# tangxyw/RecAlgorithm

Hardware: NVIDIA H100
Metric: ctr_fwd_bwd_samples_per_sec (higher is better)
Workload: dtype f32

## Files before the change

### recalgorithm_b200/csrc/ctr_common.cuh

```cuda
#pragma once
#include <cuda_runtime.h>
#include <stdint.h>
#include <stdio.h>

#include <type_traits>

#include "../../include/ctr_b200.h"

namespace ctr {

void set_error(const char* fmt, ...);
void count_launch(int n = 1);
int sm_count();

#define CTR_REQUIRE(cond, ...)                                   \
  do {                                                           \
    if (!(cond)) {                                               \
      ctr::set_error(__VA_ARGS__);                               \
      return CTR_ERR_INVALID_ARG;                                \
    }                                                            \
  } while (0)

#define CTR_UNSUPPORTED(cond, ...)                               \
  do {                                                           \
    if (cond) {                                                  \
      ctr::set_error(__VA_ARGS__);                               \
      return CTR_ERR_UNSUPPORTED;                                \
    }                                                            \
  } while (0)

#define CTR_CHECK_LAUNCH(name)                                                   \
  do {                                                                           \
    cudaError_t e__ = cudaGetLastError();                                        \
    if (e__ != cudaSuccess) {                                                    \
      ctr::set_error("%s: launch failed: %s", name, cudaGetErrorString(e__));    \
      return CTR_ERR_CUDA;                                                       \
    }                                                                            \
    ctr::count_launch();                                                         \
  } while (0)

#define CTR_CUDA(call)                                                           \
  do {                                                                           \
    cudaError_t e__ = (call);                                                    \
    if (e__ != cudaSuccess) {                                                    \
      ctr::set_error("%s failed: %s", #call, cudaGetErrorString(e__));           \
      return CTR_ERR_CUDA;                                                       \
    }                                                                            \
  } while (0)

__device__ __forceinline__ float warp_sum(float v) {
#pragma unroll
  for (int o = 16; o > 0; o >>= 1) v += __shfl_xor_sync(0xffffffffu, v, o);
  return v;
}

__device__ __forceinline__ float4 ldg_stream_f4(const float4* p) {
  float4 r;
  asm volatile("ld.global.nc.L1::no_allocate.v4.f32 {%0,%1,%2,%3}, [%4];"
               : "=f"(r.x), "=f"(r.y), "=f"(r.z), "=f"(r.w) : "l"(p));
  return r;
}
__device__ __forceinline__ void stg_stream_f4(float4* p, const float4& v) {
  asm volatile("st.global.cs.v4.f32 [%0], {%1,%2,%3,%4};" ::"l"(p), "f"(v.x), "f"(v.y), "f"(v.z), "f"(v.w)
               : "memory");
}
__device__ __forceinline__ long long ldg_stream_i64(const long long* p) {
  long long r;
  asm volatile("ld.global.nc.L1::no_allocate.s64 %0, [%1];" : "=l"(r) : "l"(p));
  return r;
}

static inline cudaStream_t as_stream(void* s) { return reinterpret_cast<cudaStream_t>(s); }
static inline bool aligned16(const void* p) { return (reinterpret_cast<uintptr_t>(p) & 15u) == 0; }

static inline int capped_grid(long long need, long long cap) { return (int)(need < cap ? need : cap); }

template <class... P, class... A>
int launch(const char* what, void (*k)(P...), dim3 grid, dim3 block, size_t smem, cudaStream_t st, const A&... args) {
  if (smem > 48 * 1024) CTR_CUDA(cudaFuncSetAttribute(k, cudaFuncAttributeMaxDynamicSharedMemorySize, (int)smem));
  k<<<grid, block, smem, st>>>(args...);
  CTR_CHECK_LAUNCH(what);
  return CTR_OK;
}

template <int MAX_PER_SM = 0, class... P, class... A>
int launch_resident(const char* what, void (*k)(P...), long long need, int block, size_t smem, cudaStream_t st,
                    const A&... args) {
  if (smem > 48 * 1024) CTR_CUDA(cudaFuncSetAttribute(k, cudaFuncAttributeMaxDynamicSharedMemorySize, (int)smem));
  int per_sm = 0;
  if (cudaOccupancyMaxActiveBlocksPerMultiprocessor(&per_sm, k, block, smem) != cudaSuccess || per_sm < 1) per_sm = 1;
  if (MAX_PER_SM > 0 && per_sm > MAX_PER_SM) per_sm = MAX_PER_SM;
  k<<<capped_grid(need, (long long)per_sm * sm_count()), block, smem, st>>>(args...);
  CTR_CHECK_LAUNCH(what);
  return CTR_OK;
}

template <int... Vs, class F>
int with_const(int v, F&& f) {
  int rc = CTR_OK;
  const bool hit = ((v == Vs && ((rc = f(std::integral_constant<int, Vs>{})), true)) || ...);
  if (!hit) {
    set_error("no kernel instantiation for %d", v);
    return CTR_ERR_INVALID_ARG;
  }
  return rc;
}
template <class F>
int with_lpr(int64_t D, F&& f) {
  return with_const<1, 2, 4, 8, 16, 32>((int)(D / 4), f);
}

}
```

### recalgorithm_b200/csrc/embed_fm2.cu

```cuda
#include "lookup_bwd.cuh"

namespace ctr {

struct PeerTables {
  const float4* base[8];
  int G, logG;
};

__device__ __forceinline__ long long load_id(const long long* p) { return ldg_stream_i64(p); }
__device__ __forceinline__ long long load_id(const int* p) {
  int r;
  asm volatile("ld.global.nc.L1::no_allocate.s32 %0, [%1];" : "=r"(r) : "l"(p));
  return (long long)r;
}
__device__ __forceinline__ float4 ld_peer_f4(const float4* p) {
  float4 r;
  asm volatile("ld.global.v4.f32 {%0,%1,%2,%3}, [%4];" : "=f"(r.x), "=f"(r.y), "=f"(r.z), "=f"(r.w) : "l"(p));
  return r;
}

template <int LPR, bool SH, int MINB, bool BI = false, typename IdT = long long, bool LIN = false, bool SEQ = false>
__global__ void __launch_bounds__(256, MINB)
embed_fm2_fwd_kernel(const float4* __restrict__ table, const PeerTables peers, const long long* __restrict__ row_off,
                     const IdT* __restrict__ ids, int B, int F, float4* __restrict__ tile,
                     float* __restrict__ fm2, long long* __restrict__ ids64_out,
                     const float4* __restrict__ wlin, float* __restrict__ lin) {
  constexpr int RPW = 32 / LPR;
  constexpr int UB = LPR < 8 ? LPR : 8;
  const unsigned full = 0xffffffffu;
  const int lane = threadIdx.x & 31;
  const int sub = lane / LPR;
  const int c = lane % LPR;
  const int warp0 = (blockIdx.x * blockDim.x + threadIdx.x) >> 5;
  const int nwarps = (gridDim.x * blockDim.x) >> 5;

  for (int b = warp0; b < B; b += nwarps) {
    float4 S = f4_zero(), Q = f4_zero();
    float lin_acc = 0.f;
    for (int f0 = 0; f0 < F; f0 += 32) {
      const int nf = min(32, F - f0);
      long long row = -1;
      if (lane < nf) {
        const long long id = load_id(ids + (size_t)b * F + f0 + lane);
        const long long lo = __ldg(row_off + (SEQ ? 0 : f0 + lane)), hi = __ldg(row_off + (SEQ ? 1 : f0 + lane + 1));
        row = (id >= 0 && id < hi - lo) ? lo + id : -1;
        if (sizeof(IdT) == 4 && ids64_out != nullptr) ids64_out[(size_t)b * F + f0 + lane] = id;
      }
#pragma unroll
      for (int it0 = 0; it0 < LPR; it0 += UB) {
        if (it0 * RPW >= nf) break;
        float4 v[UB];
        bool in[UB];
#pragma unroll
        for (int u = 0; u < UB; ++u) {
          const int fs = (it0 + u) * RPW + sub;
          const long long r = __shfl_sync(full, row, fs);
          in[u] = fs < nf;
          v[u] = f4_zero();
          if (in[u] && r >= 0) {
            if (SH) v[u] = ld_peer_f4(peers.base[r & (peers.G - 1)] + (size_t)(r >> peers.logG) * LPR + c);
            else v[u] = ldg_stream_f4(table + (size_t)r * LPR + c);
          }
        }
#pragma unroll
        for (int u = 0; u < UB; ++u) {
          S.x += v[u].x; S.y += v[u].y; S.z += v[u].z; S.w += v[u].w;
          Q.x = __fadd_rn(Q.x, __fmul_rn(v[u].x, v[u].x)); Q.y = __fadd_rn(Q.y, __fmul_rn(v[u].y, v[u].y));
          Q.z = __fadd_rn(Q.z, __fmul_rn(v[u].z, v[u].z)); Q.w = __fadd_rn(Q.w, __fmul_rn(v[u].w, v[u].w));
          if (tile != nullptr && in[u]) {
            const int fs = (it0 + u) * RPW + sub;
            stg_stream_f4(tile + ((size_t)b * F + f0 + fs) * LPR + c, v[u]);
          }
          if (LIN && in[u]) {
            const float4 w = __ldg(wlin + (size_t)(f0 + (it0 + u) * RPW + sub) * LPR + c);
            lin_acc += v[u].x * w.x + v[u].y * w.y + v[u].z * w.z + v[u].w * w.w;
          }
        }
      }
    }
    if (LIN) {
      lin_acc = warp_sum(lin_acc);
      if (lane == 0) lin[b] = lin_acc;
    }
    if (fm2 != nullptr) {
#pragma unroll
      for (int o = LPR; o < 32; o <<= 1) {
        S.x += __shfl_xor_sync(full, S.x, o); S.y += __shfl_xor_sync(full, S.y, o);
        S.z += __shfl_xor_sync(full, S.z, o); S.w += __shfl_xor_sync(full, S.w, o);
        Q.x += __shfl_xor_sync(full, Q.x, o); Q.y += __shfl_xor_sync(full, Q.y, o);
        Q.z += __shfl_xor_sync(full, Q.z, o); Q.w += __shfl_xor_sync(full, Q.w, o);
      }
      if (BI) {
        if (lane < LPR) {
          float4 r;
          r.x = 0.5f * __fsub_rn(__fmul_rn(S.x, S.x), Q.x); r.y = 0.5f * __fsub_rn(__fmul_rn(S.y, S.y), Q.y);
          r.z = 0.5f * __fsub_rn(__fmul_rn(S.z, S.z), Q.z); r.w = 0.5f * __fsub_rn(__fmul_rn(S.w, S.w), Q.w);
          reinterpret_cast<float4*>(fm2)[(size_t)b * LPR + c] = r;
        }
        continue;
      }
      float p = 0.5f * __fsub_rn(__fmul_rn(S.x, S.x), Q.x) + 0.5f * __fsub_rn(__fmul_rn(S.y, S.y), Q.y) +
                0.5f * __fsub_rn(__fmul_rn(S.z, S.z), Q.z) + 0.5f * __fsub_rn(__fmul_rn(S.w, S.w), Q.w);
#pragma unroll
      for (int o = 1; o < LPR; o <<= 1) p += __shfl_xor_sync(full, p, o);
      if (lane == 0) fm2[b] = p;
    }
  }
}

enum { FM2_PLAIN, FM2_BI, FM2_LIN };

struct StoreRow {
  float4* __restrict__ o_row;
  __device__ __forceinline__ void fetch(int, int) {}
  __device__ __forceinline__ void operator()(int, int j, const float4& r) { stg_stream_f4(o_row + j, r); }
};

template <int LPR, int HOLD, int MODE>
__global__ void __launch_bounds__(256, MODE == FM2_LIN ? 2 : 0)
embed_fm2_bwd_kernel(const float4* __restrict__ tile, const float4* __restrict__ d_tile, const float* __restrict__ d_fm2,
                     const float* __restrict__ d_lin, int B, int F, float4* __restrict__ row_grads, float4* __restrict__ d_wlin) {
  extern __shared__ float4 s_lin[];
  const int lane = threadIdx.x & 31;
  const int warp0 = (blockIdx.x * blockDim.x + threadIdx.x) >> 5;
  const int nwarps = (gridDim.x * blockDim.x) >> 5;
  const int n4 = F * LPR;
  LinHead<MODE == FM2_LIN ? HOLD : 1> lin;
  if (MODE == FM2_LIN) lin.stage(s_lin, d_tile, n4);
  for (int b = warp0; b < B; b += nwarps) {
    StoreRow sink{row_grads + (size_t)b * n4};
    RowGrad rows{d_tile ? d_tile + (size_t)b * n4 : nullptr};
    float4 g4;
    if (MODE == FM2_BI) {
      g4 = __ldg(reinterpret_cast<const float4*>(d_fm2) + (size_t)b * LPR + lane % LPR);
    } else {
      const float g = d_fm2 ? __ldg(d_fm2 + b) : 0.f;
      g4 = make_float4(g, g, g, g);
    }
    if constexpr (MODE == FM2_LIN) {
      lin.gl = d_lin ? __ldg(d_lin + b) : 0.f;
      lookup_bwd_sample<LPR, HOLD>(tile + (size_t)b * n4, n4, lane, g4, lin, sink);
    } else {
      lookup_bwd_sample<LPR, HOLD>(tile + (size_t)b * n4, n4, lane, g4, rows, sink);
    }
  }
  if (MODE == FM2_LIN) lin.flush(d_wlin, lane);
}

template <int LPR>
__global__ void __launch_bounds__(256)
embed_scatter_add_kernel(float4* __restrict__ grad_table, const long long* __restrict__ row_off,
                         const long long* __restrict__ ids, const float4* __restrict__ row_grads, int B, int F) {
  const size_t total = (size_t)B * F * LPR;
  for (size_t t = (size_t)blockIdx.x * blockDim.x + threadIdx.x; t < total; t += (size_t)gridDim.x * blockDim.x) {
    const int c = (int)(t % LPR);
    const size_t bf = t / LPR;
    const int f = (int)(bf % F);
    const long long id = __ldg(ids + bf);
    const long long lo = __ldg(row_off + f), hi = __ldg(row_off + f + 1);
    if (id >= 0 && id < hi - lo) {
      const float4 g = ldg_stream_f4(row_grads + t);
      atomicAdd(grad_table + (size_t)(lo + id) * LPR + c, g);
    }
  }
}

__global__ void __launch_bounds__(256)
bag_lookup_fwd_kernel(const float* __restrict__ table, long long V, int D, const long long* __restrict__ ids,
                      const long long* __restrict__ offsets, int B, float* __restrict__ out, long long out_stride,
                      int G) {
  const int tid = blockIdx.x * blockDim.x + threadIdx.x;
  const int gl = threadIdx.x % G;
  const int nthreads = gridDim.x * blockDim.x;
  for (int b = tid / G; b < B; b += nthreads / G) {
    const long long s = __ldg(offsets + b), e = __ldg(offsets + b + 1);
    float acc[8];
#pragma unroll
    for (int k = 0; k < 8; ++k) acc[k] = 0.f;
    int n = 0;
    for (long long i = s; i < e; ++i) {
      const long long id = __ldg(ids + i);
      if (id >= 0 && id < V) {
        ++n;
#pragma unroll
        for (int k = 0; k < 8; ++k) {
          const int dd = k * G + gl;
          if (dd < D) acc[k] += __ldg(table + (size_t)id * D + dd);
        }
      }
    }
#pragma unroll
    for (int k = 0; k < 8; ++k) {
      const int dd = k * G + gl;
      if (dd < D) out[(size_t)b * out_stride + dd] = n > 0 ? acc[k] / (float)n : 0.f;
    }
  }
}

__global__ void __launch_bounds__(256)
bag_lookup_bwd_kernel(const float* __restrict__ d_out, long long out_stride, long long V, int D,
                      const long long* __restrict__ ids, const long long* __restrict__ offsets, int B,
                      float* __restrict__ row_grads, int G) {
  const int tid = blockIdx.x * blockDim.x + threadIdx.x;
  const int gl = threadIdx.x % G;
  const int nthreads = gridDim.x * blockDim.x;
  for (int b = tid / G; b < B; b += nthreads / G) {
    const long long s = __ldg(offsets + b), e = __ldg(offsets + b + 1);
    int n = 0;
    for (long long i = s; i < e; ++i) {
      const long long id = __ldg(ids + i);
      n += (id >= 0 && id < V);
    }
    for (long long i = s; i < e; ++i) {
      const long long id = __ldg(ids + i);
      const bool ok = id >= 0 && id < V;
      for (int dd = gl; dd < D; dd += G) {
        const float g = __ldg(d_out + (size_t)b * out_stride + dd);
        row_grads[(size_t)i * D + dd] = ok ? g / (float)n : 0.f;
      }
    }
  }
}

__global__ void __launch_bounds__(256)
first_order_fwd_kernel(const float* __restrict__ w, const long long* __restrict__ row_off,
                       const long long* __restrict__ ids, int B, int F, float bias, float* __restrict__ out) {
  const int lane = threadIdx.x & 31;
  const int warp0 = (blockIdx.x * blockDim.x + threadIdx.x) >> 5;
  const int nwarps = (gridDim.x * blockDim.x) >> 5;
  for (int b = warp0; b < B; b += nwarps) {
    float acc = 0.f;
    for (int f = lane; f < F; f += 32) {
      const long long id = ldg_stream_i64(ids + (size_t)b * F + f);
      const long long lo = __ldg(row_off + f), hi = __ldg(row_off + f + 1);
      if (id >= 0 && id < hi - lo) acc += __ldg(w + lo + id);
    }
    acc = warp_sum(acc);
    if (lane == 0) out[b] = acc + bias;
  }
}

template <int LPR, typename IdT>
static int launch_fwd(const float* table, const PeerTables* peers, const int64_t* off, const IdT* ids, int64_t B,
                      int64_t F, float* tile, float* fm2, int64_t* ids64_out, cudaStream_t st) {
  PeerTables none = {};
  const PeerTables& pt = peers ? *peers : none;
  auto go = [&](auto k) {
    return launch_resident("ctr_embed_fm2_fwd", k, (B + 7) / 8, 256, 0, st, reinterpret_cast<const float4*>(table), pt,
                           reinterpret_cast<const long long*>(off), ids, (int)B, (int)F, reinterpret_cast<float4*>(tile), fm2,
                           reinterpret_cast<long long*>(ids64_out), nullptr, nullptr);
  };
  return peers != nullptr ? go(embed_fm2_fwd_kernel<LPR, true, 1, false, IdT>) : go(embed_fm2_fwd_kernel<LPR, false, 4, false, IdT>);
}

template <int MODE>
static int launch_bwd(const char* what, const float* tile, const float* d_tile, const float* d_fm2, const float* d_lin, int64_t B,
                      int64_t F, int64_t D, float* row_grads, float* d_wlin, cudaStream_t st) {
  return with_lpr(D, [&](auto LPR) {
    return with_hold<MODE != FM2_LIN>(F, LPR, [&](auto HOLD) {
      return launch_resident(what, embed_fm2_bwd_kernel<LPR, HOLD, MODE>, (B + 7) / 8, 256,
                             MODE == FM2_LIN ? sizeof(float4) * 2 * (size_t)F * LPR : 0, st, reinterpret_cast<const float4*>(tile),
                             reinterpret_cast<const float4*>(d_tile), d_fm2, d_lin, (int)B, (int)F,
                             reinterpret_cast<float4*>(row_grads), reinterpret_cast<float4*>(d_wlin));
    }, what);
  });
}

template <int LPR>
static int launch_fwd_bi(const float* table, const int64_t* off, const int64_t* ids, int64_t B, int64_t F, float* tile,
                         float* bi, cudaStream_t st) {
  return launch_resident("ctr_embed_bi_fwd", embed_fm2_fwd_kernel<LPR, false, 4, true>, (B + 7) / 8, 256, 0, st,
                         reinterpret_cast<const float4*>(table), PeerTables{}, reinterpret_cast<const long long*>(off),
                         reinterpret_cast<const long long*>(ids), (int)B, (int)F, reinterpret_cast<float4*>(tile), bi, nullptr,
                         nullptr, nullptr);
}

static int check_bfd(const char* fn, int64_t B, int64_t F, int64_t D) {
  CTR_REQUIRE(B >= 0 && F >= 1 && D >= 1, "%s: bad sizes B=%lld F=%lld D=%lld", fn, (long long)B, (long long)F,
              (long long)D);
  CTR_REQUIRE(B <= 0x7fffffffLL / 8 && F <= 65536, "%s: B=%lld / F=%lld too large", fn, (long long)B, (long long)F);
  CTR_UNSUPPORTED(D % 4 != 0 || D > 128 || (D & (D - 1)) != 0,
                  "%s: D=%lld unsupported by the fused 128-bit path (need a power of two in 4..128); "
                  "use ctr_bag_lookup_* for other widths", fn, (long long)D);
  return CTR_OK;
}

template <typename IdT>
static int dispatch_fwd(const float* table, const PeerTables* peers, const int64_t* off, const IdT* ids, int64_t B,
                        int64_t F, int64_t D, float* tile, float* fm2, int64_t* ids64_out, cudaStream_t st) {
  return with_lpr(D, [&](auto LPR) { return launch_fwd<LPR>(table, peers, off, ids, B, F, tile, fm2, ids64_out, st); });
}

static int fill_peers(const char* fn, PeerTables& peers, const float* const* shard_ptrs, int64_t G) {
  CTR_REQUIRE(G >= 1 && G <= 8 && (G & (G - 1)) == 0, "%s: G=%lld must be a power of two <= 8", fn, (long long)G);
  peers = PeerTables{};
  peers.G = (int)G;
  while ((1 << peers.logG) < G) ++peers.logG;
  for (int r = 0; r < G; ++r) {
    CTR_REQUIRE(shard_ptrs[r] != nullptr && aligned16(shard_ptrs[r]), "%s: shard %d null/unaligned", fn, r);
    peers.base[r] = reinterpret_cast<const float4*>(shard_ptrs[r]);
  }
  return CTR_OK;
}

}

using namespace ctr;

extern "C" int ctr_embed_fm2_fwd(const float* table, const int64_t* field_row_offset, const int64_t* ids,
                                 int64_t B, int64_t F, int64_t D, float* tile, float* fm2, void* stream) {
  int rc = check_bfd("ctr_embed_fm2_fwd", B, F, D);
  if (rc) return rc;
  CTR_REQUIRE(table && field_row_offset && ids, "ctr_embed_fm2_fwd: null table/field_row_offset/ids");
  CTR_REQUIRE(tile || fm2, "ctr_embed_fm2_fwd: both outputs are NULL");
  CTR_REQUIRE(aligned16(table) && aligned16(tile), "ctr_embed_fm2_fwd: table and tile must be 16-byte aligned");
  if (B == 0) return CTR_OK;
  cudaStream_t st = as_stream(stream);
  return dispatch_fwd(table, nullptr, field_row_offset, reinterpret_cast<const long long*>(ids), B, F, D, tile, fm2, nullptr, st);
}

extern "C" int ctr_embed_fm2_fwd_ids32(const float* table, const int64_t* field_row_offset, const int32_t* ids, int64_t B,
                                       int64_t F, int64_t D, float* tile, float* fm2, int64_t* ids64_out, void* stream) {
  int rc = check_bfd("ctr_embed_fm2_fwd_ids32", B, F, D);
  if (rc) return rc;
  CTR_REQUIRE(table && field_row_offset && ids, "ctr_embed_fm2_fwd_ids32: null table/field_row_offset/ids");
  CTR_REQUIRE(tile || fm2, "ctr_embed_fm2_fwd_ids32: both outputs are NULL");
  CTR_REQUIRE(aligned16(table) && aligned16(tile), "ctr_embed_fm2_fwd_ids32: table and tile must be 16-byte aligned");
  if (B == 0) return CTR_OK;
  return dispatch_fwd(table, nullptr, field_row_offset, reinterpret_cast<const int*>(ids), B, F, D, tile, fm2, ids64_out,
                      as_stream(stream));
}

extern "C" int ctr_embed_fm2_fwd_sharded(const float* const* shard_ptrs, int64_t G, const int64_t* field_row_offset,
                                         const int64_t* ids, int64_t B, int64_t F, int64_t D, float* tile, float* fm2,
                                         void* stream) {
  int rc = check_bfd("ctr_embed_fm2_fwd_sharded", B, F, D);
  if (rc) return rc;
  CTR_REQUIRE(shard_ptrs && field_row_offset && ids, "ctr_embed_fm2_fwd_sharded: null shard_ptrs/field_row_offset/ids");
  CTR_REQUIRE(tile || fm2, "ctr_embed_fm2_fwd_sharded: both outputs are NULL");
  PeerTables peers;
  rc = fill_peers("ctr_embed_fm2_fwd_sharded", peers, shard_ptrs, G);
  if (rc) return rc;
  CTR_REQUIRE(aligned16(tile), "ctr_embed_fm2_fwd_sharded: tile must be 16-byte aligned");
  if (B == 0) return CTR_OK;
  return dispatch_fwd(nullptr, &peers, field_row_offset, reinterpret_cast<const long long*>(ids), B, F, D, tile, fm2, nullptr,
                      as_stream(stream));
}

extern "C" int ctr_embed_fm2_fwd_sharded_ids32(const float* const* shard_ptrs, int64_t G, const int64_t* field_row_offset,
                                               const int32_t* ids, int64_t B, int64_t F, int64_t D, float* tile, float* fm2,
                                               int64_t* ids64_out, void* stream) {
  int rc = check_bfd("ctr_embed_fm2_fwd_sharded_ids32", B, F, D);
  if (rc) return rc;
  CTR_REQUIRE(shard_ptrs && field_row_offset && ids, "ctr_embed_fm2_fwd_sharded_ids32: null shard_ptrs/field_row_offset/ids");
  CTR_REQUIRE(tile || fm2, "ctr_embed_fm2_fwd_sharded_ids32: both outputs are NULL");
  PeerTables peers;
  rc = fill_peers("ctr_embed_fm2_fwd_sharded_ids32", peers, shard_ptrs, G);
  if (rc) return rc;
  CTR_REQUIRE(aligned16(tile), "ctr_embed_fm2_fwd_sharded_ids32: tile must be 16-byte aligned");
  if (B == 0) return CTR_OK;
  return dispatch_fwd(nullptr, &peers, field_row_offset, reinterpret_cast<const int*>(ids), B, F, D, tile, fm2, ids64_out,
                      as_stream(stream));
}

extern "C" int ctr_embed_fm2_bwd(const float* tile, const float* d_tile, const float* d_fm2, int64_t B, int64_t F,
                                 int64_t D, float* row_grads, void* stream) {
  int rc = check_bfd("ctr_embed_fm2_bwd", B, F, D);
  if (rc) return rc;
  CTR_REQUIRE(tile && row_grads, "ctr_embed_fm2_bwd: null tile/row_grads");
  CTR_REQUIRE(aligned16(tile) && aligned16(d_tile) && aligned16(row_grads),
              "ctr_embed_fm2_bwd: tile, d_tile and row_grads must be 16-byte aligned");
  if (B == 0) return CTR_OK;
  return launch_bwd<FM2_PLAIN>("ctr_embed_fm2_bwd", tile, d_tile, d_fm2, nullptr, B, F, D, row_grads, nullptr, as_stream(stream));
}

extern "C" int ctr_embed_scatter_add(float* grad_table, const int64_t* field_row_offset, const int64_t* ids,
                                     const float* row_grads, int64_t B, int64_t F, int64_t D, void* stream) {
  int rc = check_bfd("ctr_embed_scatter_add", B, F, D);
  if (rc) return rc;
  CTR_REQUIRE(grad_table && field_row_offset && ids && row_grads, "ctr_embed_scatter_add: null argument");
  CTR_REQUIRE(aligned16(grad_table) && aligned16(row_grads), "ctr_embed_scatter_add: buffers must be 16-byte aligned");
  if (B == 0) return CTR_OK;
  cudaStream_t st = as_stream(stream);
  const long long total = (long long)B * F * (D / 4);
  const int grid = capped_grid((total + 255) / 256, (long long)sm_count() * 16);
  return with_lpr(D, [&](auto LPR) {
    return launch("ctr_embed_scatter_add", embed_scatter_add_kernel<LPR>, grid, 256, 0, st, reinterpret_cast<float4*>(grad_table),
                  reinterpret_cast<const long long*>(field_row_offset), reinterpret_cast<const long long*>(ids),
                  reinterpret_cast<const float4*>(row_grads), (int)B, (int)F);
  });
}

static int bag_group(int64_t D) {
  int G = 1;
  while (G < D && G < 32) G <<= 1;
  return G;
}

extern "C" int ctr_bag_lookup_fwd(const float* table, int64_t V, int64_t D, const int64_t* ids,
                                  const int64_t* offsets, int64_t B, float* out, int64_t out_stride, void* stream) {
  CTR_REQUIRE(table && offsets && out, "ctr_bag_lookup_fwd: null argument");
  CTR_REQUIRE(B >= 0 && V >= 0 && D >= 1 && out_stride >= D, "ctr_bag_lookup_fwd: bad sizes");
  CTR_UNSUPPORTED(D > 256, "ctr_bag_lookup_fwd: D=%lld > 256", (long long)D);
  if (B == 0) return CTR_OK;
  const int G = bag_group(D);
  return launch("ctr_bag_lookup_fwd", bag_lookup_fwd_kernel, capped_grid(((long long)B * G + 255) / 256, (long long)sm_count() * 16),
                256, 0, as_stream(stream), table, V, (int)D, reinterpret_cast<const long long*>(ids),
                reinterpret_cast<const long long*>(offsets), (int)B, out, out_stride, G);
}

extern "C" int ctr_bag_lookup_bwd(const float* d_out, int64_t out_stride, int64_t V, int64_t D, const int64_t* ids,
                                  const int64_t* offsets, int64_t B, float* row_grads, void* stream) {
  CTR_REQUIRE(d_out && offsets, "ctr_bag_lookup_bwd: null argument");
  CTR_REQUIRE(B >= 0 && V >= 0 && D >= 1 && out_stride >= D, "ctr_bag_lookup_bwd: bad sizes");
  CTR_UNSUPPORTED(D > 256, "ctr_bag_lookup_bwd: D=%lld > 256", (long long)D);
  if (B == 0) return CTR_OK;
  const int G = bag_group(D);
  return launch("ctr_bag_lookup_bwd", bag_lookup_bwd_kernel, capped_grid(((long long)B * G + 255) / 256, (long long)sm_count() * 16),
                256, 0, as_stream(stream), d_out, out_stride, V, (int)D, reinterpret_cast<const long long*>(ids),
                reinterpret_cast<const long long*>(offsets), (int)B, row_grads, G);
}

extern "C" int ctr_first_order_fwd(const float* w, const int64_t* field_row_offset, const int64_t* ids, int64_t B,
                                   int64_t F, float bias, float* out, void* stream) {
  CTR_REQUIRE(w && field_row_offset && ids && out, "ctr_first_order_fwd: null argument");
  CTR_REQUIRE(B >= 0 && F >= 1 && B <= 0x7fffffffLL / 8 && F <= 65536, "ctr_first_order_fwd: bad sizes");
  if (B == 0) return CTR_OK;
  return launch("ctr_first_order_fwd", first_order_fwd_kernel, capped_grid((B + 7) / 8, (long long)sm_count() * 8), 256, 0,
                as_stream(stream), w, reinterpret_cast<const long long*>(field_row_offset), reinterpret_cast<const long long*>(ids),
                (int)B, (int)F, bias, out);
}

extern "C" int ctr_embed_bi_fwd(const float* table, const int64_t* field_row_offset, const int64_t* ids, int64_t B, int64_t F,
                                int64_t D, float* tile, float* bi, void* stream) {
  int rc = check_bfd("ctr_embed_bi_fwd", B, F, D);
  if (rc) return rc;
  CTR_REQUIRE(table && field_row_offset && ids && bi, "ctr_embed_bi_fwd: null table/field_row_offset/ids/bi");
  CTR_REQUIRE(aligned16(table) && aligned16(tile) && aligned16(bi), "ctr_embed_bi_fwd: table, tile and bi must be 16-byte aligned");
  if (B == 0) return CTR_OK;
  cudaStream_t st = as_stream(stream);
  return with_lpr(D, [&](auto LPR) { return launch_fwd_bi<LPR>(table, field_row_offset, ids, B, F, tile, bi, st); });
}

extern "C" int ctr_embed_bi_bwd(const float* tile, const float* d_tile, const float* d_bi, int64_t B, int64_t F, int64_t D,
                                float* row_grads, void* stream) {
  int rc = check_bfd("ctr_embed_bi_bwd", B, F, D);
  if (rc) return rc;
  CTR_REQUIRE(tile && d_bi && row_grads, "ctr_embed_bi_bwd: null tile/d_bi/row_grads");
  CTR_REQUIRE(aligned16(tile) && aligned16(d_tile) && aligned16(d_bi) && aligned16(row_grads),
              "ctr_embed_bi_bwd: tile, d_tile, d_bi and row_grads must be 16-byte aligned");
  if (B == 0) return CTR_OK;
  return launch_bwd<FM2_BI>("ctr_embed_fm2_bwd", tile, d_tile, d_bi, nullptr, B, F, D, row_grads, nullptr, as_stream(stream));
}

template <int LPR, typename IdT>
static int launch_fwd_lin(const float* table, const PeerTables* peers, const int64_t* off, const IdT* ids, int64_t B, int64_t F,
                          float* tile, float* fm2, int64_t* ids64_out, const float* wlin, float* lin, cudaStream_t st) {
  auto go = [&](auto k, const float4* tb, const PeerTables& pt) {
    return launch_resident("ctr_embed_fm2_lin_fwd", k, (B + 7) / 8, 256, 0, st, tb, pt, reinterpret_cast<const long long*>(off),
                           ids, (int)B, (int)F, reinterpret_cast<float4*>(tile), fm2, reinterpret_cast<long long*>(ids64_out),
                           reinterpret_cast<const float4*>(wlin), lin);
  };
  if (peers != nullptr) return go(embed_fm2_fwd_kernel<LPR, true, 1, false, IdT, true>, nullptr, *peers);
  return go(embed_fm2_fwd_kernel<LPR, false, 3, false, IdT, true>, reinterpret_cast<const float4*>(table), PeerTables{});
}

template <typename IdT>
static int dispatch_fwd_lin(const float* table, const PeerTables* peers, const int64_t* off, const IdT* ids, int64_t B, int64_t F,
                            int64_t D, float* tile, float* fm2, int64_t* ids64_out, const float* wlin, float* lin, cudaStream_t st) {
  return with_lpr(D, [&](auto LPR) { return launch_fwd_lin<LPR>(table, peers, off, ids, B, F, tile, fm2, ids64_out, wlin, lin, st); });
}

extern "C" int ctr_embed_fm2_lin_fwd(const float* table, const int64_t* field_row_offset, const void* ids, int ids_are_int32,
                                     int64_t B, int64_t F, int64_t D, const float* wlin, float* tile, float* fm2, float* lin,
                                     int64_t* ids64_out, void* stream) {
  int rc = check_bfd("ctr_embed_fm2_lin_fwd", B, F, D);
  if (rc) return rc;
  CTR_REQUIRE(table && field_row_offset && ids && wlin && lin, "ctr_embed_fm2_lin_fwd: null table/field_row_offset/ids/wlin/lin");
  CTR_REQUIRE(aligned16(table) && aligned16(tile) && aligned16(wlin), "ctr_embed_fm2_lin_fwd: table, tile and wlin must be 16-byte aligned");
  if (B == 0) return CTR_OK;
  cudaStream_t st = as_stream(stream);
  if (ids_are_int32)
    return dispatch_fwd_lin(table, nullptr, field_row_offset, reinterpret_cast<const int*>(ids), B, F, D, tile, fm2, ids64_out, wlin, lin, st);
  return dispatch_fwd_lin(table, nullptr, field_row_offset, reinterpret_cast<const long long*>(ids), B, F, D, tile, fm2, nullptr, wlin, lin, st);
}

extern "C" int ctr_embed_fm2_lin_fwd_sharded(const float* const* shard_ptrs, int64_t G, const int64_t* field_row_offset,
                                             const void* ids, int ids_are_int32, int64_t B, int64_t F, int64_t D, const float* wlin,
                                             float* tile, float* fm2, float* lin, int64_t* ids64_out, void* stream) {
  int rc = check_bfd("ctr_embed_fm2_lin_fwd_sharded", B, F, D);
  if (rc) return rc;
  CTR_REQUIRE(shard_ptrs && field_row_offset && ids && wlin && lin, "ctr_embed_fm2_lin_fwd_sharded: null argument");
  PeerTables peers;
  rc = fill_peers("ctr_embed_fm2_lin_fwd_sharded", peers, shard_ptrs, G);
  if (rc) return rc;
  CTR_REQUIRE(aligned16(tile) && aligned16(wlin), "ctr_embed_fm2_lin_fwd_sharded: tile and wlin must be 16-byte aligned");
  if (B == 0) return CTR_OK;
  cudaStream_t st = as_stream(stream);
  if (ids_are_int32)
    return dispatch_fwd_lin(nullptr, &peers, field_row_offset, reinterpret_cast<const int*>(ids), B, F, D, tile, fm2, ids64_out, wlin, lin, st);
  return dispatch_fwd_lin(nullptr, &peers, field_row_offset, reinterpret_cast<const long long*>(ids), B, F, D, tile, fm2, nullptr, wlin, lin, st);
}

extern "C" int ctr_embed_fm2_lin_bwd(const float* tile, const float* wlin, const float* d_fm2, const float* d_lin, int64_t B,
                                     int64_t F, int64_t D, float* row_grads, float* d_wlin, void* stream) {
  int rc = check_bfd("ctr_embed_fm2_lin_bwd", B, F, D);
  if (rc) return rc;
  CTR_REQUIRE(tile && wlin && row_grads && d_wlin, "ctr_embed_fm2_lin_bwd: null tile/wlin/row_grads/d_wlin");
  CTR_REQUIRE(aligned16(tile) && aligned16(wlin) && aligned16(row_grads) && aligned16(d_wlin),
              "ctr_embed_fm2_lin_bwd: buffers must be 16-byte aligned");
  cudaStream_t st = as_stream(stream);
  CTR_CUDA(cudaMemsetAsync(d_wlin, 0, sizeof(float) * F * D, st));
  if (B == 0) return CTR_OK;
  return launch_bwd<FM2_LIN>("ctr_embed_fm2_lin_bwd", tile, wlin, d_fm2, d_lin, B, F, D, row_grads, d_wlin, st);
}

template <int LPR>
static int launch_seq(const float* table, const int64_t* range2, const int64_t* ids, int64_t B, int64_t T, float* out, cudaStream_t st) {
  return launch_resident("ctr_embed_seq_fwd", embed_fm2_fwd_kernel<LPR, false, 4, false, long long, false, true>, (B + 7) / 8, 256,
                         0, st, reinterpret_cast<const float4*>(table), PeerTables{}, reinterpret_cast<const long long*>(range2),
                         reinterpret_cast<const long long*>(ids), (int)B, (int)T, reinterpret_cast<float4*>(out), nullptr, nullptr,
                         nullptr, nullptr);
}

extern "C" int ctr_embed_seq_fwd(const float* table, const int64_t* row_range, const int64_t* ids, int64_t B, int64_t T, int64_t D,
                                 float* out, void* stream) {
  int rc = check_bfd("ctr_embed_seq_fwd", B, T > 0 ? T : 1, D);
  if (rc) return rc;
  CTR_REQUIRE(table && row_range && out && (ids || B * T == 0), "ctr_embed_seq_fwd: null argument");
  CTR_REQUIRE(aligned16(table) && aligned16(out), "ctr_embed_seq_fwd: table and out must be 16-byte aligned");
  if (B == 0 || T == 0) return CTR_OK;
  cudaStream_t st = as_stream(stream);
  return with_lpr(D, [&](auto LPR) { return launch_seq<LPR>(table, row_range, ids, B, T, out, st); });
}
```

### recalgorithm_b200/csrc/lookup_bwd.cuh

```cuda
#pragma once
#include "ctr_common.cuh"

namespace ctr {

__device__ __forceinline__ float4 f4_zero() { return make_float4(0.f, 0.f, 0.f, 0.f); }

template <int LPR>
__device__ __forceinline__ void lane_group_sum(float4& v) {
#pragma unroll
  for (int o = LPR; o < 32; o <<= 1) {
    v.x += __shfl_xor_sync(0xffffffffu, v.x, o); v.y += __shfl_xor_sync(0xffffffffu, v.y, o);
    v.z += __shfl_xor_sync(0xffffffffu, v.z, o); v.w += __shfl_xor_sync(0xffffffffu, v.w, o);
  }
}

__device__ __forceinline__ float4 fm2_row_grad(const float4& dt, const float4& g, const float4& S, const float4& e) {
  float4 r;
  r.x = dt.x + g.x * (S.x - e.x); r.y = dt.y + g.y * (S.y - e.y);
  r.z = dt.z + g.z * (S.z - e.z); r.w = dt.w + g.w * (S.w - e.w);
  return r;
}

template <int HOLD, class Chunk>
__device__ __forceinline__ void load_tile_row(float4 (&e)[HOLD], const float4* __restrict__ e_row, int n4, int lane, Chunk&& chunk) {
#pragma unroll
  for (int k = 0; k < HOLD; ++k) {
    const int j = k * 32 + lane;
    e[k] = f4_zero();
    if (j < n4) {
      e[k] = ldg_stream_f4(e_row + j);
      chunk(k, j);
    }
  }
}

template <int LPR, int HOLD>
__device__ __forceinline__ float4 tile_row_sum(const float4 (&e)[HOLD]) {
  float4 S = f4_zero();
#pragma unroll
  for (int k = 0; k < HOLD; ++k) { S.x += e[k].x; S.y += e[k].y; S.z += e[k].z; S.w += e[k].w; }
  lane_group_sum<LPR>(S);
  return S;
}

struct RowGrad {
  const float4* __restrict__ row;
  __device__ __forceinline__ void load(float4& d, int j) const {
    if (row != nullptr) d = ldg_stream_f4(row + j);
  }
  __device__ __forceinline__ float4 at(int, const float4& d) const { return d; }
  __device__ __forceinline__ void add(int, const float4&) {}
};

template <int HOLD>
struct LinHead {
  static_assert(HOLD > 0, "the LIN head needs the register-resident row");
  float4* s_w;
  int n4;
  float gl;
  float4 acc[HOLD];
  __device__ __forceinline__ void stage(float4* smem, const float4* __restrict__ wlin, int n) {
    s_w = smem;
    n4 = n;
    for (int j = threadIdx.x; j < n4; j += blockDim.x) { s_w[j] = __ldg(wlin + j); s_w[n4 + j] = f4_zero(); }
    __syncthreads();
#pragma unroll
    for (int k = 0; k < HOLD; ++k) acc[k] = f4_zero();
  }
  __device__ __forceinline__ void load(float4&, int) const {}
  __device__ __forceinline__ float4 at(int j, const float4&) const {
    const float4 w = s_w[j];
    return make_float4(gl * w.x, gl * w.y, gl * w.z, gl * w.w);
  }
  __device__ __forceinline__ void add(int k, const float4& e) {
    acc[k].x += gl * e.x; acc[k].y += gl * e.y; acc[k].z += gl * e.z; acc[k].w += gl * e.w;
  }
  __device__ __forceinline__ void flush(float4* __restrict__ d_wlin, int lane) {
#pragma unroll
    for (int k = 0; k < HOLD; ++k) {
      const int j = k * 32 + lane;
      if (j < n4) {
        float* a = reinterpret_cast<float*>(s_w + n4 + j);
        atomicAdd(a + 0, acc[k].x); atomicAdd(a + 1, acc[k].y); atomicAdd(a + 2, acc[k].z); atomicAdd(a + 3, acc[k].w);
      }
    }
    __syncthreads();
    for (int j = threadIdx.x; j < n4; j += blockDim.x) atomicAdd(d_wlin + j, s_w[n4 + j]);
  }
};

template <int LPR, int HOLD, class Head, class Sink>
__device__ __forceinline__ void lookup_bwd_sample(const float4* __restrict__ e_row, int n4, int lane, const float4& g, Head& head,
                                                  Sink& sink) {
  if constexpr (HOLD > 0) {
    float4 e[HOLD], dt[HOLD];
    load_tile_row(e, e_row, n4, lane, [](int, int) {});
#pragma unroll
    for (int k = 0; k < HOLD; ++k) {
      const int j = k * 32 + lane;
      dt[k] = f4_zero();
      if (j < n4) {
        head.load(dt[k], j);
        sink.fetch(k, j);
      }
    }
    const float4 S = tile_row_sum<LPR>(e);
#pragma unroll
    for (int k = 0; k < HOLD; ++k) {
      const int j = k * 32 + lane;
      if (j < n4) {
        sink(k, j, fm2_row_grad(head.at(j, dt[k]), g, S, e[k]));
        head.add(k, e[k]);
      }
    }
  } else {
    float4 S = f4_zero();
    for (int j = lane; j < n4; j += 32) {
      const float4 v = __ldg(e_row + j);
      S.x += v.x; S.y += v.y; S.z += v.z; S.w += v.w;
    }
    lane_group_sum<LPR>(S);
    for (int j = lane; j < n4; j += 32) {
      const float4 v = __ldg(e_row + j);
      float4 dt = f4_zero();
      head.load(dt, j);
      sink(0, j, fm2_row_grad(head.at(j, dt), g, S, v));
    }
  }
}

template <bool TWO_PASS, class Fn>
int with_hold(int64_t F, int64_t LPR, Fn&& f, const char* fn = "", const char* hint = "") {
  const int64_t per_lane = (F * LPR + 31) / 32;
  if (per_lane <= 4) return f(std::integral_constant<int, 4>{});
  if (per_lane <= 8) return f(std::integral_constant<int, 8>{});
  if (per_lane <= 12) return f(std::integral_constant<int, 12>{});
  if constexpr (TWO_PASS) {
    return f(std::integral_constant<int, 0>{});
  } else {
    set_error("%s: F*D = %lld exceeds the register-resident limit of 1536%s", fn, (long long)(F * LPR * 4), hint);
    return CTR_ERR_UNSUPPORTED;
  }
}

}
```

Before: 104.1 million.

## Keep tail of forward tile in L2 and start backward from those rows

The forward kernel now writes the last batch rows of the embedding tile with normal (L2-allocating) stores and reads their table rows with evict-first loads. The number of kept rows is sized to about three quarters of the L2 capacity. The backward kernel rotates its sample order so it begins at those recently written rows, and tile loads use evict-first hints, so the tile re-read can hit in L2 instead of DRAM. This couples the forward and backward schedules and depends on the L2 size query and on nothing else evicting the kept region between the two kernels.

```diff
diff --git a/recalgorithm_b200/csrc/ctr_common.cuh b/recalgorithm_b200/csrc/ctr_common.cuh
--- a/recalgorithm_b200/csrc/ctr_common.cuh
+++ b/recalgorithm_b200/csrc/ctr_common.cuh
@@ -60,6 +60,11 @@
                : "=f"(r.x), "=f"(r.y), "=f"(r.z), "=f"(r.w) : "l"(p));
   return r;
 }
+__device__ __forceinline__ float4 ldg_once_f4(const float4* p) {
+  float4 r;
+  asm volatile("ld.global.cs.nc.v4.f32 {%0,%1,%2,%3}, [%4];" : "=f"(r.x), "=f"(r.y), "=f"(r.z), "=f"(r.w) : "l"(p));
+  return r;
+}
 __device__ __forceinline__ void stg_stream_f4(float4* p, const float4& v) {
   asm volatile("st.global.cs.v4.f32 [%0], {%1,%2,%3,%4};" ::"l"(p), "f"(v.x), "f"(v.y), "f"(v.z), "f"(v.w)
                : "memory");
diff --git a/recalgorithm_b200/csrc/embed_fm2.cu b/recalgorithm_b200/csrc/embed_fm2.cu
--- a/recalgorithm_b200/csrc/embed_fm2.cu
+++ b/recalgorithm_b200/csrc/embed_fm2.cu
@@ -24,9 +24,10 @@
 embed_fm2_fwd_kernel(const float4* __restrict__ table, const PeerTables peers, const long long* __restrict__ row_off,
                      const IdT* __restrict__ ids, int B, int F, float4* __restrict__ tile,
                      float* __restrict__ fm2, long long* __restrict__ ids64_out,
-                     const float4* __restrict__ wlin, float* __restrict__ lin) {
+                     const float4* __restrict__ wlin, float* __restrict__ lin, int keep_from) {
   constexpr int RPW = 32 / LPR;
   constexpr int UB = LPR < 8 ? LPR : 8;
+  constexpr bool KEEP = LPR <= 8 && !SH && !BI && !LIN && !SEQ;
   const unsigned full = 0xffffffffu;
   const int lane = threadIdx.x & 31;
   const int sub = lane / LPR;
@@ -35,6 +36,7 @@
   const int nwarps = (gridDim.x * blockDim.x) >> 5;
 
   for (int b = warp0; b < B; b += nwarps) {
+    const bool keep = KEEP && b >= keep_from;
     float4 S = f4_zero(), Q = f4_zero();
     float lin_acc = 0.f;
     for (int f0 = 0; f0 < F; f0 += 32) {
@@ -59,7 +61,7 @@
           v[u] = f4_zero();
           if (in[u] && r >= 0) {
             if (SH) v[u] = ld_peer_f4(peers.base[r & (peers.G - 1)] + (size_t)(r >> peers.logG) * LPR + c);
-            else v[u] = ldg_stream_f4(table + (size_t)r * LPR + c);
+            else v[u] = keep ? ldg_once_f4(table + (size_t)r * LPR + c) : ldg_stream_f4(table + (size_t)r * LPR + c);
           }
         }
 #pragma unroll
@@ -69,7 +71,9 @@
           Q.z = __fadd_rn(Q.z, __fmul_rn(v[u].z, v[u].z)); Q.w = __fadd_rn(Q.w, __fmul_rn(v[u].w, v[u].w));
           if (tile != nullptr && in[u]) {
             const int fs = (it0 + u) * RPW + sub;
-            stg_stream_f4(tile + ((size_t)b * F + f0 + fs) * LPR + c, v[u]);
+            float4* p = tile + ((size_t)b * F + f0 + fs) * LPR + c;
+            if (keep) *p = v[u];
+            else stg_stream_f4(p, v[u]);
           }
           if (LIN && in[u]) {
             const float4 w = __ldg(wlin + (size_t)(f0 + (it0 + u) * RPW + sub) * LPR + c);
@@ -119,7 +123,8 @@
 template <int LPR, int HOLD, int MODE>
 __global__ void __launch_bounds__(256, MODE == FM2_LIN ? 2 : 0)
 embed_fm2_bwd_kernel(const float4* __restrict__ tile, const float4* __restrict__ d_tile, const float* __restrict__ d_fm2,
-                     const float* __restrict__ d_lin, int B, int F, float4* __restrict__ row_grads, float4* __restrict__ d_wlin) {
+                     const float* __restrict__ d_lin, int B, int F, float4* __restrict__ row_grads, float4* __restrict__ d_wlin,
+                     int first) {
   extern __shared__ float4 s_lin[];
   const int lane = threadIdx.x & 31;
   const int warp0 = (blockIdx.x * blockDim.x + threadIdx.x) >> 5;
@@ -127,7 +132,8 @@
   const int n4 = F * LPR;
   LinHead<MODE == FM2_LIN ? HOLD : 1> lin;
   if (MODE == FM2_LIN) lin.stage(s_lin, d_tile, n4);
-  for (int b = warp0; b < B; b += nwarps) {
+  for (int i = warp0; i < B; i += nwarps) {
+    const int b = HOLD == 0 ? i : i < B - first ? i + first : i - (B - first);
     StoreRow sink{row_grads + (size_t)b * n4};
     RowGrad rows{d_tile ? d_tile + (size_t)b * n4 : nullptr};
     float4 g4;
@@ -240,15 +246,23 @@
   }
 }
 
+static int keep_from(int64_t B, int64_t F, int64_t D) {
+  int dev = 0, l2 = 0;
+  if (cudaGetDevice(&dev) != cudaSuccess || cudaDeviceGetAttribute(&l2, cudaDevAttrL2CacheSize, dev) != cudaSuccess) l2 = 0;
+  const long long n = (long long)l2 * 3 / 4 / (F * D * (long long)sizeof(float));
+  return (int)(B - (n < B ? n : B));
+}
+
 template <int LPR, typename IdT>
 static int launch_fwd(const float* table, const PeerTables* peers, const int64_t* off, const IdT* ids, int64_t B,
                       int64_t F, float* tile, float* fm2, int64_t* ids64_out, cudaStream_t st) {
   PeerTables none = {};
   const PeerTables& pt = peers ? *peers : none;
+  const int keep = peers != nullptr ? (int)B : keep_from(B, F, LPR * 4);
   auto go = [&](auto k) {
     return launch_resident("ctr_embed_fm2_fwd", k, (B + 7) / 8, 256, 0, st, reinterpret_cast<const float4*>(table), pt,
                            reinterpret_cast<const long long*>(off), ids, (int)B, (int)F, reinterpret_cast<float4*>(tile), fm2,
-                           reinterpret_cast<long long*>(ids64_out), nullptr, nullptr);
+                           reinterpret_cast<long long*>(ids64_out), nullptr, nullptr, keep);
   };
   return peers != nullptr ? go(embed_fm2_fwd_kernel<LPR, true, 1, false, IdT>) : go(embed_fm2_fwd_kernel<LPR, false, 4, false, IdT>);
 }
@@ -261,7 +275,8 @@
       return launch_resident(what, embed_fm2_bwd_kernel<LPR, HOLD, MODE>, (B + 7) / 8, 256,
                              MODE == FM2_LIN ? sizeof(float4) * 2 * (size_t)F * LPR : 0, st, reinterpret_cast<const float4*>(tile),
                              reinterpret_cast<const float4*>(d_tile), d_fm2, d_lin, (int)B, (int)F,
-                             reinterpret_cast<float4*>(row_grads), reinterpret_cast<float4*>(d_wlin));
+                             reinterpret_cast<float4*>(row_grads), reinterpret_cast<float4*>(d_wlin),
+                             MODE == FM2_PLAIN && HOLD > 0 ? keep_from(B, F, D) : 0);
     }, what);
   });
 }
@@ -272,7 +287,7 @@
   return launch_resident("ctr_embed_bi_fwd", embed_fm2_fwd_kernel<LPR, false, 4, true>, (B + 7) / 8, 256, 0, st,
                          reinterpret_cast<const float4*>(table), PeerTables{}, reinterpret_cast<const long long*>(off),
                          reinterpret_cast<const long long*>(ids), (int)B, (int)F, reinterpret_cast<float4*>(tile), bi, nullptr,
-                         nullptr, nullptr);
+                         nullptr, nullptr, (int)B);
 }
 
 static int check_bfd(const char* fn, int64_t B, int64_t F, int64_t D) {
@@ -459,7 +474,7 @@
   auto go = [&](auto k, const float4* tb, const PeerTables& pt) {
     return launch_resident("ctr_embed_fm2_lin_fwd", k, (B + 7) / 8, 256, 0, st, tb, pt, reinterpret_cast<const long long*>(off),
                            ids, (int)B, (int)F, reinterpret_cast<float4*>(tile), fm2, reinterpret_cast<long long*>(ids64_out),
-                           reinterpret_cast<const float4*>(wlin), lin);
+                           reinterpret_cast<const float4*>(wlin), lin, (int)B);
   };
   if (peers != nullptr) return go(embed_fm2_fwd_kernel<LPR, true, 1, false, IdT, true>, nullptr, *peers);
   return go(embed_fm2_fwd_kernel<LPR, false, 3, false, IdT, true>, reinterpret_cast<const float4*>(table), PeerTables{});
@@ -520,7 +535,7 @@
   return launch_resident("ctr_embed_seq_fwd", embed_fm2_fwd_kernel<LPR, false, 4, false, long long, false, true>, (B + 7) / 8, 256,
                          0, st, reinterpret_cast<const float4*>(table), PeerTables{}, reinterpret_cast<const long long*>(range2),
                          reinterpret_cast<const long long*>(ids), (int)B, (int)T, reinterpret_cast<float4*>(out), nullptr, nullptr,
-                         nullptr, nullptr);
+                         nullptr, nullptr, (int)B);
 }
 
 extern "C" int ctr_embed_seq_fwd(const float* table, const int64_t* row_range, const int64_t* ids, int64_t B, int64_t T, int64_t D,
diff --git a/recalgorithm_b200/csrc/lookup_bwd.cuh b/recalgorithm_b200/csrc/lookup_bwd.cuh
--- a/recalgorithm_b200/csrc/lookup_bwd.cuh
+++ b/recalgorithm_b200/csrc/lookup_bwd.cuh
@@ -28,7 +28,7 @@
     const int j = k * 32 + lane;
     e[k] = f4_zero();
     if (j < n4) {
-      e[k] = ldg_stream_f4(e_row + j);
+      e[k] = ldg_once_f4(e_row + j);
       chunk(k, j);
     }
   }
@@ -46,7 +46,7 @@
 struct RowGrad {
   const float4* __restrict__ row;
   __device__ __forceinline__ void load(float4& d, int j) const {
-    if (row != nullptr) d = ldg_stream_f4(row + j);
+    if (row != nullptr) d = ldg_once_f4(row + j);
   }
   __device__ __forceinline__ float4 at(int, const float4& d) const { return d; }
   __device__ __forceinline__ void add(int, const float4&) {}
```

Result: no change. 104.4 million, median of 6 (+0.4%).
